# duxfrederic/lightcurver

Measured on AMD Instinct MI355X. Metric: cutouts/sec (PSF-fit + joint forward-model iter), 32x32 & 64x64 stamps, higher is better.
Workload: dtype f32

## Files before the change

lightcurver_amd/csrc/psf_kernels.h:

```cpp
#pragma once
#include <type_traits>
#include <utility>

#include "lc_common.h"
#include "starlet_device.h"

#ifndef LC_XPOLL_SLEEP
#define LC_XPOLL_SLEEP 2
#endif
#ifndef LC_P5_AHEAD
#define LC_P5_AHEAD 1
#endif
#ifndef LC_STARLET_LIVE_ADDR
#define LC_STARLET_LIVE_ADDR 1
#endif
#ifndef LC_SERIAL_TRIM
#define LC_SERIAL_TRIM 1
#endif
#ifndef LC_TASK_AHEAD
#define LC_TASK_AHEAD 1
#endif
#ifndef LC_V_ZERO_ONCE
#define LC_V_ZERO_ONCE LC_TASK_AHEAD
#endif
#ifndef LC_LOOP_ONLY
#define LC_LOOP_ONLY 1
#endif
#ifndef LC_LOOP_TOP_LIVE
#define LC_LOOP_TOP_LIVE 1
#endif
namespace lc {
constexpr int kXFlagStride = 16;

#ifdef LC_STAMPS
__device__ long long g_stamps[128];
#define LC_STAMP(k)                                                      \
  do {                                                                   \
    if ((blockIdx.x == 0 || blockIdx.x == 8) && threadIdx.x == 0 && it == A.n_iter - 1)  \
      g_stamps[(k) + (blockIdx.x == 8 ? 64 : 0)] = clock64();            \
  } while (0)
#else
#define LC_STAMP(k) do {} while (0)
#endif


struct PsfArgs {
  int F, S, n_iter, t0, hist_stride, mode;
  const float *data, *wgt;
  const float *W;
  const float *norms;
  const float *Tm;
  float *B, *mB, *sB;
  float *stars, *stars_m, *stars_s;
  float *hist;
  float *qscratch;
  float *out_loss, *out_chi2, *out_gstars, *out_ggrid, *out_gT, *out_model;
  float lam_sc, lam_hf;
  lc_adabelief_cfg ab;
  float *xch;
  int *xflags, *xabort;
  int launch_seq, heal, force_abort_it;
  const float *bkB, *bkmB, *bksB, *bkstars, *bkstars_m, *bkstars_s;
  int *heal_count;
  const float *ext_grad;
  const float *sched;
  float *B1, *mB1, *sB1;
  int xcd_fast;
};

typedef float lc_v4f __attribute__((ext_vector_type(4)));
__device__ __forceinline__ void store_sc1_x4(float *p, lc_v4f v) {
  asm volatile("global_store_dwordx4 %0, %1, off sc1\n\ts_nop 2" ::"v"(p), "v"(v) : "memory");
}
__device__ __forceinline__ void store_plain_x4(float *p, lc_v4f v) {
  asm volatile("global_store_dwordx4 %0, %1, off\n\ts_nop 2" ::"v"(p), "v"(v) : "memory");
}
__device__ __forceinline__ void store_sc1_f(float *p, float v) {
  asm volatile("global_store_dword %0, %1, off sc1" ::"v"(p), "v"(v) : "memory");
}
__device__ __forceinline__ void load_sc1_2x4(const float *p, lc_v4f &a, lc_v4f &b) {
  asm volatile("global_load_dwordx4 %0, %2, off sc1\n\tglobal_load_dwordx4 %1, %2, off offset:16 sc1\n\ts_waitcnt vmcnt(0)"
               : "=&v"(a), "=&v"(b)
               : "v"(p)
               : "memory");
}
__device__ __forceinline__ void load_sc1_2x4_1(const float *p, lc_v4f &a, lc_v4f &b, const float *ps, float &s) {
  asm volatile("global_load_dword %2, %4, off sc1\n\tglobal_load_dwordx4 %0, %3, off sc1\n\tglobal_load_dwordx4 %1, %3, off offset:16 sc1\n\ts_waitcnt vmcnt(0)"
               : "=&v"(a), "=&v"(b), "=&v"(s)
               : "v"(p), "v"(ps)
               : "memory");
}
__device__ __forceinline__ void load_sc1_x4(const float *p, lc_v4f &a) {
  asm volatile("global_load_dwordx4 %0, %1, off sc1\n\ts_waitcnt vmcnt(0)" : "=&v"(a) : "v"(p) : "memory");
}
__device__ __forceinline__ float load_sc1_f(const float *p) {
  float v;
  asm volatile("global_load_dword %0, %1, off sc1\n\ts_waitcnt vmcnt(0)" : "=&v"(v) : "v"(p) : "memory");
  return v;
}


template <int N_, int SS_, int PX_, int SG_, bool WC_ = false, int JB_ = 8>
struct PsfCfg {
  static constexpr int N = N_, SS = SS_, PX = PX_, SG = SG_;
  static constexpr bool WC = WC_;
  static constexpr bool SPLIT_LOOP_ONLY = (N == 32 || N == 64);
  static constexpr int n = N / SS;
  static constexpr int NTHR = N * N / PX;
  static constexpr int NW = (NTHR + kWave - 1) / kWave;
  static constexpr int NT = ntaps(SS);
  static constexpr int J = ilog2(N);
  static constexpr int LR = 8;
  static constexpr int LC = (JB_ * (N_ / SS_) / 4 >= 64) ? 4 : 2;
  static constexpr int LA = LC;
  static constexpr int TS = N + 1;
  static constexpr int RS = n + 1;
  static constexpr int OFF_T = 0;
  static constexpr int SZ_T = WC_ ? N * (N + 2 * (N / 4 + 10) + 1) : N * TS;
  static constexpr int OFF_R = OFF_T + SZ_T;
  static constexpr int SZ_R2 = SG * n * TS;
  static constexpr int VS = WC_ ? n + 3 : RS, VO = WC_ ? 1 : 0;
  static constexpr int SZ_V = SG * N * VS;
  static constexpr int JB = JB_;
  static constexpr int AP = N / 4 + 10;
  static constexpr int TSA = N + 2 * AP + 1;
  static constexpr int APR = AP / SS + 2;
  static constexpr int JBP = JB + 1;
  static constexpr int WSZ = JB * TSA + (n + 2 * APR) * JBP;
  static constexpr int SZ_VR = (SZ_V > StarletLds<N>::FLOATS) ? SZ_V : StarletLds<N>::FLOATS;
  static constexpr int OFF_WSC = OFF_R + SZ_VR;
  static constexpr int SZ_R = WC ? (SZ_VR + NW * WSZ) : ((2 * SZ_R2 > SZ_V) ? 2 * SZ_R2 : SZ_V);
  static constexpr int OFF_RES = OFF_R + SZ_R;
  static constexpr int SZ_RES = WC ? 0 : SG * n * n;
  static constexpr int OFF_TAPS = OFF_RES + SZ_RES;
  static constexpr int NTP = NT + 3;
  static constexpr int SZ_TAPS = (16 * 4 * NTP + 1) / 2 * 2 + 16 * 2 * NT * 2;
  static constexpr int OFF_TAPP = OFF_TAPS + (16 * 4 * NTP + 1) / 2 * 2;
  static constexpr int OFF_RED = OFF_TAPS + SZ_TAPS;
  static constexpr int IPS = n * n / LC;
  static constexpr int IPS_PAD = (IPS + kWave - 1) / kWave * kWave;
  static constexpr int SLOTS = IPS_PAD / kWave;
  static constexpr int SZ_REDX = 16 * NW;
  static constexpr int SZ_RED = (WC ? 16 * (n / JB) * 5 : SG * SLOTS * 5) + SZ_REDX + NW + 8;
  static constexpr int OFF_REDX = OFF_RED + (WC ? 16 * (n / JB) * 5 : SG * SLOTS * 5);
  static constexpr int OFF_REDW = OFF_REDX + SZ_REDX;
  static constexpr int OFF_STAR = OFF_RED + SZ_RED;
  static constexpr int MAXS = 16;
  static constexpr int SZ_STAR = MAXS * 20 + 16;
  static constexpr int LDS_FLOATS = OFF_STAR + SZ_STAR;
  static_assert(WC || StarletLds<N>::FLOATS <= SZ_T + SZ_R + SZ_RES, "starlet ping-pong buffers must fit over T + R + RES");
  static_assert(PX % SS == 0 && N % PX == 0 && n % LR == 0 && n % LC == 0 && n % LA == 0 && n % JB == 0, "tiling");
  static_assert(LDS_FLOATS * 4 <= 163840, "LDS");
  static_assert(OFF_TAPP % 2 == 0, "tap pairs are read as 64-bit words");
  static_assert(NTHR <= 1024 && NTHR % kWave == 0, "threads");
  static_assert(!WC_ || PX_ <= 8, "the WC layout keeps the pixel state in registers");
};


template <int SS, int NT>
__device__ inline void tap_entry(float delta, int k, float &tap, float &dtap, int &bq) {
  const int o = (int)nearbyintf(delta);
  const int base = o - kRg - (SS - 1);
  int q = base / SS;
  if (q * SS > base) --q;
  bq = q;
  const int m = q * SS + k;
  const float inv_s2 = 1.0f / (kSigmaG * kSigmaG);
  const float nrm = 0.3989422804014327f / kSigmaG;
  float a = 0.f, d = 0.f;
#pragma unroll
  for (int dv = 0; dv < SS; ++dv) {
    const int t = m + dv;
    if (t >= o - kRg && t <= o + kRg) {
      const float x = (float)t - delta;
      const float p = nrm * expf(-0.5f * x * x * inv_s2);
      a += p;
      d += p * x * inv_s2;
    }
  }
  tap = a;
  dtap = d;
}

template <class C, bool SPLIT = false>
__global__ __launch_bounds__(C::NTHR) void psf_fit_kernel(PsfArgs A) {
  constexpr int N = C::N, SS = C::SS, PX = C::PX, SG = C::SG, n = C::n, NT = C::NT, J = C::J;
  constexpr int NTHR = C::NTHR, TS = C::TS, RS = C::RS, LR = C::LR, LC = C::LC, LA = C::LA;
  extern __shared__ __align__(16) float lds[];
  float *T = lds + C::OFF_T;
  float *R2t = lds + C::OFF_R;
  float *R2xt = R2t + C::SZ_R2;
  float *V = lds + C::OFF_R;
  float *RES = lds + C::OFF_RES;
  float *TAPS = lds + C::OFF_TAPS + 1;
  constexpr int NTP = C::NTP;
  lc_v2f *TAPP = (lc_v2f *)(lds + C::OFF_TAPP);
  float *REDX = lds + C::OFF_REDX;
  float *RED = lds + C::OFF_RED;
  float *REDW = lds + C::OFF_REDW;
  float *SCAL = REDW + C::NW;
  float *SP = lds + C::OFF_STAR;
  float *SGR = SP + C::MAXS * 4;
  float *SM = SGR + C::MAXS * 5;
  float *SV = SM + C::MAXS * 4;
  int *BQ = (int *)(SV + C::MAXS * 4);

  int f = blockIdx.x, role = 0;
  if constexpr (SPLIT) {
    f = ((int)blockIdx.x >> 4) * 8 + ((int)blockIdx.x & 7);
    role = ((int)blockIdx.x >> 3) & 1;
    if (f >= A.F) return;
  }
  const bool conv_role = !SPLIT || role == 0, starlet_role = !SPLIT || role == 1;
  const int my_xcc = SPLIT ? (int)(__builtin_amdgcn_s_getreg(20 | (3 << 11)) & 15u) : 0;
  int same_xcd = 0;
  const int tid0 = threadIdx.x;
  const int S = A.S;
  constexpr bool LOOP_ONLY = SPLIT && LC_LOOP_ONLY && C::SPLIT_LOOP_ONLY;
  const bool loop = LOOP_ONLY || A.mode == 1;

  const float *dataf = A.data + (size_t)f * S * n * n;
  const float *wgtf = A.wgt + (size_t)f * S * n * n;

  if constexpr (!SPLIT) {
    if (A.heal) {
      if (__hip_atomic_load(A.xabort, __ATOMIC_RELAXED, __HIP_MEMORY_SCOPE_AGENT) != A.launch_seq) return;
      const size_t o = (size_t)f * N * N;
      for (int i = tid0; i < N * N; i += NTHR) {
        A.B[o + i] = A.bkB[o + i];
        A.mB[o + i] = A.bkmB[o + i];
        A.sB[o + i] = A.bksB[o + i];
      }
      if (tid0 < S * 4) {
        A.stars[(size_t)f * S * 4 + tid0] = A.bkstars[(size_t)f * S * 4 + tid0];
        A.stars_m[(size_t)f * S * 4 + tid0] = A.bkstars_m[(size_t)f * S * 4 + tid0];
        A.stars_s[(size_t)f * S * 4 + tid0] = A.bkstars_s[(size_t)f * S * 4 + tid0];
      }
      if (f == 0 && tid0 == 0) atomicAdd(A.heal_count, 1);
      __threadfence_block();
      __syncthreads();
    }
  }

  if constexpr (C::WC) {
    for (int i = tid0; i < C::SZ_T; i += NTHR) lds[C::OFF_T + i] = 0.f;
    for (int i = tid0; i < C::NW * C::WSZ; i += NTHR) lds[C::OFF_WSC + i] = 0.f;
  }
  if (tid0 < S * 4) {
    SP[tid0] = A.stars[(size_t)f * S * 4 + tid0];
    SM[tid0] = A.stars_m[(size_t)f * S * 4 + tid0];
    SV[tid0] = A.stars_s[(size_t)f * S * 4 + tid0];
  }
  __syncthreads();

  constexpr bool STATE_REGS = (PX <= 8);
  float *Bg = A.B, *mBg = A.mB, *sBg = A.sB;
  if constexpr (SPLIT && !STATE_REGS) {
    if (role == 1) {
      const size_t g0pix = (size_t)f * N * N + (size_t)(tid0 / (N / PX)) * N + (tid0 % (N / PX)) * PX;
#pragma unroll
      for (int q = 0; q < PX / 4; ++q) {
        ((float4 *)(A.B1 + g0pix))[q] = ((const float4 *)(A.B + g0pix))[q];
        ((float4 *)(A.mB1 + g0pix))[q] = ((const float4 *)(A.mB + g0pix))[q];
        ((float4 *)(A.sB1 + g0pix))[q] = ((const float4 *)(A.sB + g0pix))[q];
      }
      Bg = A.B1;
      mBg = A.mB1;
      sBg = A.sB1;
    }
  }
  float Bp[PX], Mp[PX], Sp_[PX], Tp[PX];
  {
    const size_t g0pix = (size_t)f * N * N + (size_t)(tid0 / (N / PX)) * N + (tid0 % (N / PX)) * PX;
#pragma unroll
    for (int q = 0; q < PX / 4; ++q) {
      if (STATE_REGS) {
        const float4 b = ((const float4 *)(A.B + g0pix))[q], t = ((const float4 *)(A.Tm + g0pix))[q];
        const float4 m = ((const float4 *)(A.mB + g0pix))[q], sv = ((const float4 *)(A.sB + g0pix))[q];
        Bp[4 * q] = b.x; Bp[4 * q + 1] = b.y; Bp[4 * q + 2] = b.z; Bp[4 * q + 3] = b.w;
        Tp[4 * q] = t.x; Tp[4 * q + 1] = t.y; Tp[4 * q + 2] = t.z; Tp[4 * q + 3] = t.w;
        Mp[4 * q] = m.x; Mp[4 * q + 1] = m.y; Mp[4 * q + 2] = m.z; Mp[4 * q + 3] = m.w;
        Sp_[4 * q] = sv.x; Sp_[4 * q + 1] = sv.y; Sp_[4 * q + 2] = sv.z; Sp_[4 * q + 3] = sv.w;
      }
    }
  }

  auto compute_taps = [&](int tid) {
    for (int e = tid; e < S * 2 * NTP; e += NTHR) {
      const int s = e / (2 * NTP), ax = (e / NTP) & 1, k = e % NTP - 1;
      float tap = 0.f, dtap = 0.f;
      int bq = 0;
      const float c_off = (N % 2 == 0) ? 0.5f : 0.0f;
      const float delta = fminf(fmaxf(SS * SP[s * 4 + 1 + ax], -(float)(N / 4)), (float)(N / 4)) + c_off;
      if (k >= 0 && k < NT) tap_entry<SS, NT>(delta, k, tap, dtap, bq);
      TAPS[(s * 4 + 2 * ax) * NTP + k] = tap;
      TAPS[(s * 4 + 2 * ax + 1) * NTP + k] = dtap;
      if (k >= 0 && k < NT) TAPP[(s * 2 + ax) * NT + k] = (lc_v2f){tap, dtap};
      if (k == 0) BQ[s * 2 + ax] = bq;
    }
  };
  auto step_stars = [&](int tid) {
#pragma clang fp contract(off)
    if (tid < S * 3) {
      const float lr = SCAL[0], bc1 = SCAL[1], bc2 = SCAL[2];
      const float b1 = A.ab.b1, b2 = A.ab.b2, eps = A.ab.eps, eps_root = A.ab.eps_root;
      const int s = tid / 3, q = tid % 3;
      const float g = SGR[s * 5 + 1 + q];
      const float mn = b1 * SM[s * 4 + q] + (1.f - b1) * g;
      const float dg = g - mn;
      const float sn = b2 * SV[s * 4 + q] + (1.f - b2) * dg * dg + eps_root;
      SM[s * 4 + q] = mn;
      SV[s * 4 + q] = sn;
      SP[s * 4 + q] -= lr * (mn * bc1) / (sqrtf(sn * bc2) + eps);
    }
  };
  auto update_stars_and_taps = [&](int tid) {
    step_stars(tid);
    __syncthreads();
    compute_taps(tid);
  };
  if (conv_role) compute_taps(tid0);
  constexpr bool TRIM = SPLIT && C::WC && PX == 8 && LC_SERIAL_TRIM;
  static_assert(!TRIM || 3 * C::MAXS <= kWave, "the x0 sums and the stars' step are lanes of one wave");
  [[maybe_unused]] float tpix_next[TRIM ? PX : 1];
  constexpr bool C2_SPLIT = SPLIT && C::WC && PX == 8;
  constexpr bool TASK_AHEAD = C2_SPLIT && LC_TASK_AHEAD, V_ZERO_ONCE = C2_SPLIT && LC_V_ZERO_ONCE;
  constexpr bool TOP_LIVE = C2_SPLIT && LOOP_ONLY && LC_LOOP_TOP_LIVE;
  if constexpr (V_ZERO_ONCE) {
    if (role == 0) {
      for (int i = tid0; i < SG * N; i += NTHR) {
        V[i * C::VS] = 0.f;
        V[i * C::VS + n + 1] = 0.f;
      }
    }
  }
  if constexpr (TRIM) {
    if (role == 0) {
      const int pu = tid0 / (N / PX), pv = (tid0 % (N / PX)) * PX;
#pragma unroll
      for (int p = 0; p < PX; ++p) {
        tpix_next[p] = Bp[p] + Tp[p];
        T[pu * C::TSA + C::AP + pv + p] = tpix_next[p];
      }
    }
    __syncthreads();
  }
  for (int it = 0; it < A.n_iter; ++it) {
    const int tglob = A.t0 + it;
    if constexpr (SPLIT) {
      if (A.force_abort_it == it && f == 0 && role == 1) {
        if (tid0 == 0) __hip_atomic_store(A.xabort, A.launch_seq, __ATOMIC_RELAXED, __HIP_MEMORY_SCOPE_AGENT);
        break;
      }
    }
    int tid = tid0;
    LC_LAUNDER(tid);
    const int lane = tid & 63, wid = tid >> 6;
    const int pu = tid / (N / PX);
    const int pv = (tid % (N / PX)) * PX;
    const size_t gpix = (size_t)f * N * N + (size_t)pu * N + pv;
    const int tid_c = TOP_LIVE ? tid0 : tid, lane_c = tid_c & 63, wid_c = tid_c >> 6;
    const int pu_c = tid_c / (N / PX), pv_c = (tid_c % (N / PX)) * PX;
    if (tid < 3 && loop) SCAL[tid] = A.sched[3 * tglob + tid];
    LC_STAMP(0);
    float gB[PX];
#pragma unroll
    for (int p = 0; p < PX; ++p) gB[p] = 0.f;
    float tpix[PX];
    if (conv_role) {
    if constexpr (TRIM) {
#pragma unroll
      for (int p = 0; p < PX; ++p) tpix[p] = tpix_next[p];
    } else if (C::WC && STATE_REGS) {
#pragma unroll
      for (int p = 0; p < PX; ++p) {
        tpix[p] = Bp[p] + Tp[p];
        T[pu_c * C::TSA + C::AP + pv_c + p] = tpix[p];
      }
    } else if (STATE_REGS) {
#pragma unroll
      for (int p = 0; p < PX; ++p) T[pu_c * TS + pv_c + p] = Bp[p] + Tp[p];
    } else {
      const float4 *bp = (const float4 *)(Bg + gpix);
      const float4 *tp = (const float4 *)(A.Tm + gpix);
#pragma unroll
      for (int q = 0; q < PX / 4; ++q) {
        const float4 b = bp[q], t = tp[q];
        T[pu_c * TS + pv_c + 4 * q + 0] = b.x + t.x;
        T[pu_c * TS + pv_c + 4 * q + 1] = b.y + t.y;
        T[pu_c * TS + pv_c + 4 * q + 2] = b.z + t.z;
        T[pu_c * TS + pv_c + 4 * q + 3] = b.w + t.w;
      }
    }
    if constexpr (!TOP_LIVE)
      if (tid_c < S * 5) SGR[tid_c] = 0.f;

    for (int g0 = 0; g0 < S; g0 += SG) {
      if (!TRIM || g0 > 0) __syncthreads();
      LC_STAMP(1 + 5 * (g0 / SG));
      if constexpr (C::WC) {
        constexpr int JB = C::JB, NBLK = n / JB;
        float *wsc = lds + C::OFF_WSC + wid_c * C::WSZ;
        constexpr int TSA = C::TSA, AP = C::AP, APR = C::APR;
        float *R2w = wsc + AP, *RESw = wsc + JB * TSA + APR * C::JBP;
        if constexpr (TASK_AHEAD) {
          static_assert(SS == 2 && N == kWave && JB * (n / LC) == kWave && LA == LC, "one item per lane in each pass of a task");
          constexpr int NP = (NT + 1) / 2, WL2 = (JB - 1) + NP, WL = SS * (LC - 1) + NT, WI = (SS * LA - 1 + NT - 1) / SS + 1;
          const int jl = lane_c % JB, a0 = (lane_c / JB) * LC;
          const int ntask = min(SG, S - g0) * NBLK;
          float dpre[LC], wpre[LC];
          lc_v2f tr2[NP], win2[WL2];
          lc_v2f py[NP];
          float rv[WI];
          auto pixel_request = [&](int task) {
            const int s = g0 + task / NBLK, jd0 = (task % NBLK) * JB;
#pragma unroll
            for (int j = 0; j < LC; ++j) {
              const size_t pix = (size_t)s * n * n + (size_t)(a0 + j) * n + jd0 + jl;
              dpre[j] = dataf[pix];
              wpre[j] = wgtf[pix];
            }
          };
          auto row_request = [&](int task, int bqx) {
            const int s = g0 + task / NBLK, jd0 = (task % NBLK) * JB;
            const float *tx = TAPS + (s * 4 + 0) * NTP;
#pragma unroll
            for (int h = 0; h < NP; ++h) tr2[h] = (lc_v2f){tx[NT - 1 - 2 * h], tx[NT - 2 - 2 * h]};
            const float *trow = T + lane_c * TSA + AP + SS * (jd0 - bqx) - (NT - 1);
#pragma unroll
            for (int i = 0; i < WL2; ++i) win2[i] = (lc_v2f){trow[2 * i], trow[2 * i + 1]};
          };
          auto row_fma_store = [&] {
            lc_v2f acc[JB];
#pragma unroll
            for (int j = 0; j < JB; ++j) acc[j] = (lc_v2f){0.f, 0.f};
#pragma unroll
            for (int h = 0; h < NP; ++h) {
#pragma unroll
              for (int j = 0; j < JB; ++j) acc[j] = pk_fma(tr2[h], win2[j + h], acc[j]);
            }
#pragma unroll
            for (int j = 0; j < JB; ++j) R2w[j * TSA + lane_c] = acc[j].x + acc[j].y;
          };
          auto tcol_request = [&](int task, int bqy) {
            const float *ty = TAPS + ((g0 + task / NBLK) * 4 + 2) * NTP;
#pragma unroll
            for (int q = 0; q < NP; ++q) py[q] = (lc_v2f){ty[2 * q], ty[2 * q - 1]};
            const float *rcol = RESw + (bqy + a0) * C::JBP + jl;
#pragma unroll
            for (int i = 0; i < WI; ++i) rv[i] = rcol[i * C::JBP];
          };
          auto tcol_fma_store = [&](int task) {
            const int sl = task / NBLK, jd0 = (task % NBLK) * JB;
            lc_v2f out2[LA];
#pragma unroll
            for (int h = 0; h < LA; ++h) out2[h] = (lc_v2f){0.f, 0.f};
#pragma unroll
            for (int i = 0; i < WI; ++i) {
              const lc_v2f rr = pk_bcast(rv[i]);
#pragma unroll
              for (int h = 0; h < LA; ++h)
                if (i - h >= 0 && i - h < NP) out2[h] = pk_fma(py[i - h], rr, out2[h]);
            }
            float *vrow = V + (sl * N + SS * a0) * C::VS + C::VO + jd0 + jl;
#pragma unroll
            for (int h = 0; h < LA; ++h) {
              vrow[(2 * h) * C::VS] = out2[h].x;
              vrow[(2 * h + 1) * C::VS] = out2[h].y;
            }
            if constexpr (!V_ZERO_ONCE) {
              if (jd0 + jl == 0) {
#pragma unroll
                for (int r = 0; r < SS * LA; ++r) V[(sl * N + SS * a0 + r) * C::VS] = 0.f;
              }
              if (jd0 + jl == n - 1) {
#pragma unroll
                for (int r = 0; r < SS * LA; ++r) V[(sl * N + SS * a0 + r) * C::VS + n + 1] = 0.f;
              }
            }
          };
// ... 492 lines not shown
              const lc_v2f vv = pk_bcast(use.vwin[i]);
#pragma unroll
              for (int k = 0; k < NT; ++k) {
                const int rel = SS * i - k;
                if (rel >= 0 && rel < PX) accp[rel] = pk_fma(use.txd[k], vv, accp[rel]);
              }
            }
            float gxs = 0.f;
#pragma unroll
            for (int p = 0; p < PX; ++p) {
              gB[p] = fmaf(use.amp, accp[p].x, gB[p]);
              gxs = fmaf(accp[p].y, tpix[p], gxs);
            }
            gxs = wave_sum(gxs);
            if (lane_c == 0) REDX[s * C::NW + wid_c] = gxs;
          };
          auto nothing = [] {};
          auto p5_window = [&](int sl, P5Ops &o, int bq) {
            o.amp = SP[(g0 + sl) * 4 + 0];
            const float *vrow = V + (sl * N + pu_c) * C::VS + 1;
            const int jd0 = bq + pv_c / SS;
#pragma unroll
            for (int i = 0; i < WJ; ++i) o.vwin[i] = vrow[min(max(jd0 + i, -1), n)];
            __builtin_amdgcn_sched_barrier(0);
          };
          auto p5_taps = [&](int sl, P5Ops &o) {
            __builtin_amdgcn_sched_barrier(0);
#pragma unroll
            for (int k = 0; k < NT; ++k) o.txd[k] = TAPP[((g0 + sl) * 2 + 0) * NT + k];
            __builtin_amdgcn_sched_barrier(0);
          };
          const int ns = min(SG, S - g0);
          P5Ops opsA, opsB;
          int bqn = BQ[min(g0 + 1, S - 1) * 2 + 0];
          p5_window(0, opsA, BQ[g0 * 2 + 0]);
          p5_taps(0, opsA);
          int sl = 0;
#pragma clang loop unroll(disable)
          while (sl + 1 < ns) {
            progress_prio((4 * sl) / SG);
            const int bqnn = BQ[min(g0 + sl + 2, S - 1) * 2 + 0];
            p5_window(sl + 1, opsB, bqn);
            p5_star(sl, opsA, [&] { p5_taps(sl + 1, opsB); });
            if (sl + 2 >= ns) {
              opsA = opsB;
              sl += 1;
              break;
            }
            bqn = BQ[min(g0 + sl + 3, S - 1) * 2 + 0];
            p5_window(sl + 2, opsA, bqnn);
            p5_star(sl + 1, opsB, [&] { p5_taps(sl + 2, opsA); });
            sl += 2;
          }
          progress_prio((4 * sl) / SG);
          p5_star(sl, opsA, nothing);
        } else {
          for (int sl = 0; sl < SG; ++sl) {
            const int s = g0 + sl;
            if (s >= S) break;
            progress_prio((4 * sl) / SG);
            const int bq = BQ[s * 2 + 0];
            const float amp = SP[s * 4 + 0];
            lc_v2f txd[NT];
#pragma unroll
            for (int k = 0; k < NT; ++k) txd[k] = TAPP[(s * 2 + 0) * NT + k];
            lc_v2f accp[PX];
#pragma unroll
            for (int p = 0; p < PX; ++p) accp[p] = (lc_v2f){0.f, 0.f};
            const float *vrow = V + (sl * N + pu_c) * C::VS + 1;
            const int jd0 = bq + pv_c / SS;
            float vwin[WJ];
#pragma unroll
            for (int i = 0; i < WJ; ++i) vwin[i] = vrow[min(max(jd0 + i, -1), n)];
#pragma unroll
            for (int i = 0; i < WJ; ++i) {
              const lc_v2f vv = pk_bcast(vwin[i]);
#pragma unroll
              for (int k = 0; k < NT; ++k) {
                const int rel = SS * i - k;
                if (rel >= 0 && rel < PX) accp[rel] = pk_fma(txd[k], vv, accp[rel]);
              }
            }
            float gxs = 0.f;
#pragma unroll
            for (int p = 0; p < PX; ++p) {
              gB[p] = fmaf(amp, accp[p].x, gB[p]);
              gxs = fmaf(accp[p].y, tpix[p], gxs);
            }
            gxs = wave_sum(gxs);
            if (lane_c == 0) REDX[s * C::NW + wid_c] = gxs;
          }
        }
        __builtin_amdgcn_s_setprio(0);
      } else {
        constexpr int WJ = (PX - 1 + NT - 1) / SS + 1;
        for (int sl = 0; sl < SG; ++sl) {
          const int s = g0 + sl;
          if (s >= S) break;
          const float *tx = TAPS + (s * 4 + 0) * NTP, *dtx = tx + NTP;
          const int bq = BQ[s * 2 + 0];
          const float amp = SP[s * 4 + 0];
          float acc[PX], gxs = 0.f;
#pragma unroll
          for (int p = 0; p < PX; ++p) acc[p] = 0.f;
#pragma unroll
          for (int i = 0; i < WJ; ++i) {
            const int jd = i + bq + pv_c / SS;
            const int ci = min(max(jd, 0), n - 1);
            float vv = V[(sl * N + pu_c) * RS + ci];
            vv = (jd >= 0 && jd < n) ? vv : 0.f;
            float dsum = 0.f;
#pragma unroll
            for (int k = 0; k < NT; ++k) {
              const int rel = SS * i - k;
              if (rel >= 0 && rel < PX) {
                acc[rel] = fmaf(tx[k], vv, acc[rel]);
                dsum = fmaf(dtx[k], T[pu_c * TS + pv_c + rel], dsum);
              }
            }
            gxs = fmaf(vv, dsum, gxs);
          }
#pragma unroll
          for (int p = 0; p < PX; ++p) gB[p] = fmaf(amp, acc[p], gB[p]);
          gxs = wave_sum(gxs);
          if (lane_c == 0) REDX[s * C::NW + wid_c] = gxs;
        }
      }
      LC_STAMP(17);
    }
    if (A.ext_grad) {
#pragma unroll
      for (int p = 0; p < PX; ++p) gB[p] += A.ext_grad[gpix + p];
    }
    }
    if constexpr (TRIM) {
      if (role == 0) {
        LC_STAMP(41);
        float *mine = A.xch + (((size_t)f * 2 + (it & 1)) * 2 + 0) * (N * N + 64);
#pragma unroll
        for (int q = 0; q < PX / 4; ++q) {
          lc_v4f v;
          v.x = gB[4 * q];
          v.y = gB[4 * q + 1];
          v.z = gB[4 * q + 2];
          v.w = gB[4 * q + 3];
          if (same_xcd) store_plain_x4(mine + pu_c * N + pv_c + 4 * q, v);
          else store_sc1_x4(mine + pu_c * N + pv_c + 4 * q, v);
        }
        if (tid_c == 0 && it == 0) store_sc1_f(mine + N * N + 1, __int_as_float(my_xcc + 1));
      }
    }
    __syncthreads();
    LC_STAMP(40);
    {
      if (conv_role && tid < S) {
        float acc = 0.f;
#pragma unroll
        for (int w = 0; w < C::NW; ++w) acc += REDX[tid * C::NW + w];
        SGR[tid * 5 + 2] = acc * SP[tid * 4 + 0] * SS;
      }
    }

    if constexpr (!LOOP_ONLY) {
      if (A.out_gT) {
#pragma unroll
        for (int p = 0; p < PX; ++p) A.out_gT[gpix + p] = gB[p];
      }
    }

    float l1 = 0.f;
    float z[PX];
#pragma unroll
    for (int p = 0; p < PX; ++p) z[p] = 0.f;
    if (starlet_role && (LOOP_ONLY || A.lam_sc != 0.f || A.lam_hf != 0.f)) {
      float bpix[PX];
      if (STATE_REGS) {
#pragma unroll
        for (int p = 0; p < PX; ++p) bpix[p] = Bp[p];
      } else {
        const float4 *bp = (const float4 *)(Bg + gpix);
#pragma unroll
        for (int q = 0; q < PX / 4; ++q) {
          const float4 b = bp[q];
          bpix[4 * q] = b.x;
          bpix[4 * q + 1] = b.y;
          bpix[4 * q + 2] = b.z;
          bpix[4 * q + 3] = b.w;
        }
      }
      constexpr bool LIVE_ADDR = SPLIT && STATE_REGS && LC_STARLET_LIVE_ADDR;
      starlet_l1_grad<N, PX, ilog2(N), LIVE_ADDR>(bpix, A.W ? A.W + (size_t)f * J * N * N : nullptr, A.norms,
                                                  A.qscratch + (size_t)f * J * N * N, A.lam_sc, A.lam_hf,
                                                  C::WC ? lds + C::OFF_R : lds, tid, l1, z);
    }
    LC_STAMP(42);
    if (!TRIM || role == 1) {
      {
        const float wl = wave_sum(l1);
        if (lane == 0) REDW[wid] = wl;
      }
      __syncthreads();
    }
    float tl1 = 0.f;
    if (tid == 0 && starlet_role)
      for (int w = 0; w < C::NW; ++w) tl1 += REDW[w];
    LC_STAMP(44);
    if constexpr (SPLIT) {
      constexpr int XS = N * N + 64;
      float *mine = A.xch + (((size_t)f * 2 + (it & 1)) * 2 + role) * XS;
      const float *theirs = A.xch + (((size_t)f * 2 + (it & 1)) * 2 + (1 - role)) * XS;
      const int poff = pu * N + pv;
      if (!TRIM || role == 1) {
#pragma unroll
      for (int q = 0; q < PX / 4; ++q) {
        lc_v4f v;
        v.x = role ? z[4 * q] : gB[4 * q];
        v.y = role ? z[4 * q + 1] : gB[4 * q + 1];
        v.z = role ? z[4 * q + 2] : gB[4 * q + 2];
        v.w = role ? z[4 * q + 3] : gB[4 * q + 3];
        if (same_xcd) store_plain_x4(mine + poff + 4 * q, v);
        else store_sc1_x4(mine + poff + 4 * q, v);
      }
      if (tid == 0 && role == 1) {
        if (same_xcd) asm volatile("global_store_dword %0, %1, off" ::"v"(mine + N * N), "v"(tl1) : "memory");
        else store_sc1_f(mine + N * N, tl1);
      }
      if (tid == 0 && it == 0) store_sc1_f(mine + N * N + 1, __int_as_float(my_xcc + 1));
      }
      constexpr bool TAPS_LATE = STATE_REGS;
      if (role == 0 && loop) {
        if constexpr (TRIM) wave_lds_sync();
        if (TAPS_LATE) step_stars(tid);
        else update_stars_and_taps(tid);
      }
      asm volatile("s_waitcnt vmcnt(0)" ::: "memory");
      __syncthreads();
      LC_STAMP(45);
      int *OK = (int *)(SCAL + 5);
      if (tid == 0) {
        if (same_xcd) asm volatile("global_store_dword %0, %1, off" ::"v"(A.xflags + ((size_t)f * 2 + role) * kXFlagStride), "v"(it + 1) : "memory");
        else __hip_atomic_store(A.xflags + ((size_t)f * 2 + role) * kXFlagStride, it + 1, __ATOMIC_RELAXED, __HIP_MEMORY_SCOPE_AGENT);
        int ok = 1, spins = 0;
        while (__hip_atomic_load(A.xflags + ((size_t)f * 2 + (1 - role)) * kXFlagStride, __ATOMIC_RELAXED, __HIP_MEMORY_SCOPE_AGENT) < it + 1) {
          __builtin_amdgcn_s_sleep(LC_XPOLL_SLEEP);
          ++spins;
          if (spins > (1 << 21) ||
              ((spins & 255) == 0 && __hip_atomic_load(A.xabort, __ATOMIC_RELAXED, __HIP_MEMORY_SCOPE_AGENT) == A.launch_seq)) {
            __hip_atomic_store(A.xabort, A.launch_seq, __ATOMIC_RELAXED, __HIP_MEMORY_SCOPE_AGENT);
            ok = 0;
            break;
          }
        }
        if (it == 0 && ok) OK[1] = (A.xcd_fast && __float_as_int(load_sc1_f(theirs + N * N + 1)) == my_xcc + 1) ? 1 : 0;
        *OK = ok;
#ifdef LC_XCH_ACQUIRE
        __builtin_amdgcn_fence(__ATOMIC_ACQUIRE, "agent");
        asm volatile("s_waitcnt vmcnt(0)" ::: "memory");
#endif
      }
      if (TAPS_LATE && role == 0 && loop) compute_taps((tid + NTHR / 2) % NTHR);
      __syncthreads();
      LC_STAMP(46);
      if (*OK == 0) break;
      if (it == 0) same_xcd = OK[1];
      float other[PX];
      float tl1_other = 0.f;
      if constexpr (PX == 8) {
        lc_v4f a, b;
        load_sc1_2x4_1(theirs + poff, a, b, theirs + N * N, tl1_other);
        other[0] = a.x; other[1] = a.y; other[2] = a.z; other[3] = a.w;
        other[4] = b.x; other[5] = b.y; other[6] = b.z; other[7] = b.w;
      } else {
#pragma unroll
        for (int q = 0; q < PX / 4; ++q) {
          lc_v4f a;
          load_sc1_x4(theirs + poff + 4 * q, a);
          other[4 * q] = a.x; other[4 * q + 1] = a.y; other[4 * q + 2] = a.z; other[4 * q + 3] = a.w;
        }
      }
#pragma unroll
      for (int p = 0; p < PX; ++p) {
        if (role) gB[p] = other[p]; else z[p] = other[p];
      }
      if (tid == 0 && role == 0) tl1 = (PX == 8) ? tl1_other : load_sc1_f(theirs + N * N);
      LC_STAMP(47);
    }
    if (!TRIM && tid == 0 && conv_role) {
      float chi = 0.f;
      for (int s = 0; s < S; ++s) chi += SGR[s * 5];
      const float loss = 0.5f * chi + tl1;
      A.hist[(size_t)f * A.hist_stride + tglob] = loss;
      if constexpr (!LOOP_ONLY) {
        if (A.out_loss) A.out_loss[f] = loss;
        if (A.out_chi2) A.out_chi2[f] = chi;
      }
    }
    if constexpr (!LOOP_ONLY) {
      if (A.out_ggrid) {
#pragma unroll
        for (int p = 0; p < PX; ++p) A.out_ggrid[gpix + p] = gB[p] + z[p];
      }
      if (A.out_gstars && tid < S * 4) {
        const int s = tid / 4, q = tid % 4;
        A.out_gstars[(size_t)f * S * 4 + tid] = SGR[s * 5 + 1 + q];
      }
    }
    if (loop) {
#pragma clang fp contract(off)
      const float lr = SCAL[0], bc1 = SCAL[1], bc2 = SCAL[2];
      const float b1 = A.ab.b1, b2 = A.ab.b2, eps = A.ab.eps, eps_root = A.ab.eps_root;
      if (STATE_REGS) {
#pragma unroll
        for (int p = 0; p < PX; ++p) {
          const float g = gB[p] + z[p];
          const float mn = b1 * Mp[p] + (1.f - b1) * g;
          const float dg = g - mn;
          const float sn = b2 * Sp_[p] + (1.f - b2) * dg * dg + eps_root;
          Mp[p] = mn;
          Sp_[p] = sn;
          Bp[p] -= lr * (mn * bc1) * __builtin_amdgcn_rcpf(__builtin_amdgcn_sqrtf(sn * bc2) + eps);
        }
      }
      if constexpr (!STATE_REGS) {
        float4 *bp = (float4 *)(Bg + gpix);
        float4 *mp = (float4 *)(mBg + gpix);
        float4 *sp = (float4 *)(sBg + gpix);
        float4 bq[PX / 4], mq[PX / 4], sq[PX / 4];
#pragma unroll
        for (int q = 0; q < PX / 4; ++q) {
          bq[q] = bp[q];
          mq[q] = mp[q];
          sq[q] = sp[q];
        }
#pragma unroll
        for (int q = 0; q < PX / 4; ++q) {
          float *bb = &bq[q].x, *mm = &mq[q].x, *ss_ = &sq[q].x;
#pragma unroll
          for (int e = 0; e < 4; ++e) {
            const float g = gB[4 * q + e] + z[4 * q + e];
            const float mn = b1 * mm[e] + (1.f - b1) * g;
            const float dg = g - mn;
            const float sn = b2 * ss_[e] + (1.f - b2) * dg * dg + eps_root;
            mm[e] = mn;
            ss_[e] = sn;
            bb[e] -= lr * (mn * bc1) * __builtin_amdgcn_rcpf(__builtin_amdgcn_sqrtf(sn * bc2) + eps);
          }
        }
#pragma unroll
        for (int q = 0; q < PX / 4; ++q) {
          bp[q] = bq[q];
          mp[q] = mq[q];
          sp[q] = sq[q];
        }
      }
      if constexpr (!SPLIT) update_stars_and_taps(tid);
    }
    if constexpr (TRIM) {
      if (role == 0) {
#pragma unroll
        for (int p = 0; p < PX; ++p) {
          tpix_next[p] = Bp[p] + Tp[p];
          T[pu_c * C::TSA + C::AP + pv_c + p] = tpix_next[p];
        }
        if (tid_c == 0) {
          float chi = 0.f;
          for (int s = 0; s < S; ++s) chi += SGR[s * 5];
          const float loss = 0.5f * chi + tl1;
          A.hist[(size_t)f * A.hist_stride + tglob] = loss;
          if constexpr (!LOOP_ONLY) {
            if (A.out_loss) A.out_loss[f] = loss;
            if (A.out_chi2) A.out_chi2[f] = chi;
          }
        }
      }
    }
    __syncthreads();
    LC_STAMP(43);
  }

  if (loop && STATE_REGS && conv_role) {
    const size_t g0pix = (size_t)f * N * N + (size_t)(tid0 / (N / PX)) * N + (tid0 % (N / PX)) * PX;
#pragma unroll
    for (int q = 0; q < PX / 4; ++q) {
      ((float4 *)(A.B + g0pix))[q] = make_float4(Bp[4 * q], Bp[4 * q + 1], Bp[4 * q + 2], Bp[4 * q + 3]);
      ((float4 *)(A.mB + g0pix))[q] = make_float4(Mp[4 * q], Mp[4 * q + 1], Mp[4 * q + 2], Mp[4 * q + 3]);
      ((float4 *)(A.sB + g0pix))[q] = make_float4(Sp_[4 * q], Sp_[4 * q + 1], Sp_[4 * q + 2], Sp_[4 * q + 3]);
    }
  }
  if (loop && tid0 < S * 4 && conv_role) {
    A.stars[(size_t)f * S * 4 + tid0] = SP[tid0];
    A.stars_m[(size_t)f * S * 4 + tid0] = SM[tid0];
    A.stars_s[(size_t)f * S * 4 + tid0] = SV[tid0];
// ... 5 lines not shown
```

lightcurver_amd/csrc/starlet_device.h:

```cpp
#pragma once
#include <utility>

#include "lc_common.h"

namespace lc {

__device__ __forceinline__ void progress_prio(int k) {
#ifndef LC_NO_PROGRESS_PRIO
  if (k <= 0) __builtin_amdgcn_s_setprio(3);
  else if (k == 1) __builtin_amdgcn_s_setprio(2);
  else if (k == 2) __builtin_amdgcn_s_setprio(1);
  else __builtin_amdgcn_s_setprio(0);
#endif
}
__device__ __forceinline__ void progress_prio_end(int done, int total) {
#ifndef LC_NO_PROGRESS_PRIO
  const int left = total - 1 - done;
  if (left >= 3) __builtin_amdgcn_s_setprio(3);
  else if (left == 2) __builtin_amdgcn_s_setprio(2);
  else if (left == 1) __builtin_amdgcn_s_setprio(1);
  else __builtin_amdgcn_s_setprio(0);
#endif
}

// ... 410 lines not shown
template <int LPR>
__device__ __forceinline__ float swz_line_last(float v) {
  constexpr int pat = ((~(LPR - 1)) & 0x1F) | ((LPR - 1) << 5);
  return __builtin_bit_cast(float, __builtin_amdgcn_ds_swizzle(__builtin_bit_cast(int, v), pat));
}
#define LC_TAP1(a, o, c, dir, k) \
  "v_fmac_f32_dpp %" #a ", %" #o ", %" #c " " dir ":%" #k " row_mask:0xf bank_mask:0xf bound_ctrl:1\n\t"
#define LC_TAP2(c, dir, k) LC_TAP1(0, 2, c, dir, k) LC_TAP1(1, 3, c, dir, k)
#define LC_TAP4(c, dir, k) LC_TAP1(0, 4, c, dir, k) LC_TAP1(1, 5, c, dir, k) LC_TAP1(2, 6, c, dir, k) LC_TAP1(3, 7, c, dir, k)
#define LC_TAP8(c, dir, k)                                                                                        \
  LC_TAP1(0, 8, c, dir, k) LC_TAP1(1, 9, c, dir, k) LC_TAP1(2, 10, c, dir, k) LC_TAP1(3, 11, c, dir, k)             \
  LC_TAP1(4, 12, c, dir, k) LC_TAP1(5, 13, c, dir, k) LC_TAP1(6, 14, c, dir, k) LC_TAP1(7, 15, c, dir, k)
#define LC_MUL1(w, o, c, dir) "v_mul_f32_dpp %" #w ", %" #o ", %" #c " " dir ":1 row_mask:0xf bank_mask:0xf bound_ctrl:1\n\t"
template <int K1, int K2>
__device__ __forceinline__ void dpp_taps(float (&acc)[2], const float (&own)[2], float cl1, float cu1, float cl2, float cu2) {
  asm("s_nop 1\n\t" LC_TAP2(4, "row_shr", 8) LC_TAP2(5, "row_shl", 8) LC_TAP2(6, "row_shr", 9) LC_TAP2(7, "row_shl", 9)
      : "+v"(acc[0]), "+v"(acc[1])
      : "v"(own[0]), "v"(own[1]), "v"(cl1), "v"(cu1), "v"(cl2), "v"(cu2), "n"(K1), "n"(K2));
}
template <int K1>
__device__ __forceinline__ void dpp_taps(float (&acc)[2], const float (&own)[2], float cl1, float cu1) {
  asm("s_nop 1\n\t" LC_TAP2(4, "row_shr", 6) LC_TAP2(5, "row_shl", 6)
      : "+v"(acc[0]), "+v"(acc[1])
      : "v"(own[0]), "v"(own[1]), "v"(cl1), "v"(cu1), "n"(K1));
}
template <int K1, int K2>
__device__ __forceinline__ void dpp_taps(float (&acc)[4], const float (&own)[4], float cl1, float cu1, float cl2, float cu2) {
  asm("s_nop 1\n\t" LC_TAP4(8, "row_shr", 12) LC_TAP4(9, "row_shl", 12) LC_TAP4(10, "row_shr", 13) LC_TAP4(11, "row_shl", 13)
      : "+v"(acc[0]), "+v"(acc[1]), "+v"(acc[2]), "+v"(acc[3])
      : "v"(own[0]), "v"(own[1]), "v"(own[2]), "v"(own[3]), "v"(cl1), "v"(cu1), "v"(cl2), "v"(cu2), "n"(K1), "n"(K2));
}
template <int K1>
__device__ __forceinline__ void dpp_taps(float (&acc)[4], const float (&own)[4], float cl1, float cu1) {
  asm("s_nop 1\n\t" LC_TAP4(8, "row_shr", 10) LC_TAP4(9, "row_shl", 10)
      : "+v"(acc[0]), "+v"(acc[1]), "+v"(acc[2]), "+v"(acc[3])
      : "v"(own[0]), "v"(own[1]), "v"(own[2]), "v"(own[3]), "v"(cl1), "v"(cu1), "n"(K1));
}
template <int K1, int K2>
__device__ __forceinline__ void dpp_taps(float (&acc)[8], const float (&own)[8], float cl1, float cu1, float cl2, float cu2) {
  asm("s_nop 1\n\t" LC_TAP8(16, "row_shr", 20) LC_TAP8(17, "row_shl", 20) LC_TAP8(18, "row_shr", 21) LC_TAP8(19, "row_shl", 21)
      : "+v"(acc[0]), "+v"(acc[1]), "+v"(acc[2]), "+v"(acc[3]), "+v"(acc[4]), "+v"(acc[5]), "+v"(acc[6]), "+v"(acc[7])
      : "v"(own[0]), "v"(own[1]), "v"(own[2]), "v"(own[3]), "v"(own[4]), "v"(own[5]), "v"(own[6]), "v"(own[7]), "v"(cl1),
        "v"(cu1), "v"(cl2), "v"(cu2), "n"(K1), "n"(K2));
}
template <int K1>
__device__ __forceinline__ void dpp_taps(float (&acc)[8], const float (&own)[8], float cl1, float cu1) {
  asm("s_nop 1\n\t" LC_TAP8(16, "row_shr", 18) LC_TAP8(17, "row_shl", 18)
      : "+v"(acc[0]), "+v"(acc[1]), "+v"(acc[2]), "+v"(acc[3]), "+v"(acc[4]), "+v"(acc[5]), "+v"(acc[6]), "+v"(acc[7])
      : "v"(own[0]), "v"(own[1]), "v"(own[2]), "v"(own[3]), "v"(own[4]), "v"(own[5]), "v"(own[6]), "v"(own[7]), "v"(cl1),
        "v"(cu1), "n"(K1));
}
template <bool SHR>
__device__ __forceinline__ void dpp_gated(float *w, const float *in, float gate, std::integral_constant<int, 2>) {
  if constexpr (SHR)
    asm("s_nop 1\n\t" LC_MUL1(0, 2, 4, "row_shr") LC_MUL1(1, 3, 4, "row_shr") : "=&v"(w[0]), "=&v"(w[1]) : "v"(in[0]), "v"(in[1]), "v"(gate));
  else
    asm("s_nop 1\n\t" LC_MUL1(0, 2, 4, "row_shl") LC_MUL1(1, 3, 4, "row_shl") : "=&v"(w[0]), "=&v"(w[1]) : "v"(in[0]), "v"(in[1]), "v"(gate));
}
#define LC_MUL4(dir) LC_MUL1(0, 4, 8, dir) LC_MUL1(1, 5, 8, dir) LC_MUL1(2, 6, 8, dir) LC_MUL1(3, 7, 8, dir)
template <bool SHR>
__device__ __forceinline__ void dpp_gated(float *w, const float *in, float gate, std::integral_constant<int, 4>) {
  if constexpr (SHR)
    asm("s_nop 1\n\t" LC_MUL4("row_shr") : "=&v"(w[0]), "=&v"(w[1]), "=&v"(w[2]), "=&v"(w[3]) : "v"(in[0]), "v"(in[1]), "v"(in[2]), "v"(in[3]), "v"(gate));
  else
    asm("s_nop 1\n\t" LC_MUL4("row_shl") : "=&v"(w[0]), "=&v"(w[1]), "=&v"(w[2]), "=&v"(w[3]) : "v"(in[0]), "v"(in[1]), "v"(in[2]), "v"(in[3]), "v"(gate));
}
#undef LC_MUL4
#define LC_MUL8(dir)                                                                                \
  LC_MUL1(0, 8, 16, dir) LC_MUL1(1, 9, 16, dir) LC_MUL1(2, 10, 16, dir) LC_MUL1(3, 11, 16, dir)       \
  LC_MUL1(4, 12, 16, dir) LC_MUL1(5, 13, 16, dir) LC_MUL1(6, 14, 16, dir) LC_MUL1(7, 15, 16, dir)
#define LC_MUL8_OPS                                                                                                      \
  : "=&v"(w[0]), "=&v"(w[1]), "=&v"(w[2]), "=&v"(w[3]), "=&v"(w[4]), "=&v"(w[5]), "=&v"(w[6]), "=&v"(w[7])                 \
  : "v"(in[0]), "v"(in[1]), "v"(in[2]), "v"(in[3]), "v"(in[4]), "v"(in[5]), "v"(in[6]), "v"(in[7]), "v"(gate)
template <bool SHR>
__device__ __forceinline__ void dpp_gated(float *w, const float *in, float gate, std::integral_constant<int, 8>) {
  if constexpr (SHR) asm("s_nop 1\n\t" LC_MUL8("row_shr") LC_MUL8_OPS);
  else asm("s_nop 1\n\t" LC_MUL8("row_shl") LC_MUL8_OPS);
}
#undef LC_MUL8_OPS
#undef LC_MUL8
#undef LC_MUL1
#undef LC_TAP8
#undef LC_TAP4
#undef LC_TAP2
#undef LC_TAP1

template <int N, int PX, int LPR, int D, bool ADJ>
__device__ __forceinline__ void line_pass(const float (&own)[PX], const LineLane &L, float (&out)[PX]) {
  constexpr float b0 = 0.375f, b1 = 0.25f, b2 = 0.0625f;
  const int lil = L.lil;
  if constexpr (D >= PX) {
    constexpr int K1 = D / PX, K2 = 2 * D / PX;
    const float cl1 = (K1 < LPR && lil >= K1) ? b1 : 0.f, cu1 = (K1 < LPR && lil + K1 < LPR) ? b1 : 0.f;
    const float cl2 = (K2 < LPR && lil >= K2) ? b2 : 0.f, cu2 = (K2 < LPR && lil + K2 < LPR) ? b2 : 0.f;
    const float ef = ((lil < K1) ? b1 : 0.f) + ((lil < K2) ? b2 : 0.f);
    const float el = ((lil + K1 >= LPR) ? b1 : 0.f) + ((lil + K2 >= LPR) ? b2 : 0.f);
    float e = 0.f;
    if constexpr (!ADJ) e = fmaf(ef, swz_line_first<LPR>(own[0]), el * swz_line_last<LPR>(own[PX - 1]));
#pragma unroll
    for (int p = 0; p < PX; ++p) out[p] = fmaf(b0, own[p], e);
    if constexpr (K2 < LPR) dpp_taps<K1, K2>(out, own, cl1, cu1, cl2, cu2);
    else if constexpr (K1 < LPR) dpp_taps<K1>(out, own, cl1, cu1);
    if constexpr (ADJ) {
      float full = own[0];
#pragma unroll
      for (int p = 1; p < PX; ++p) full += own[p];
      const float hs = line_sum<LPR>(full * ef), ts = line_sum<LPR>(full * el);
      out[0] = fmaf(L.is_first, hs, out[0]);
      out[PX - 1] = fmaf(L.is_last, ts, out[PX - 1]);
    }
  } else {
    static_assert(2 * D <= PX, "dilations below PX reach the adjacent lane only");
    const float has_lower = 1.f - L.is_first, has_upper = 1.f - L.is_last;
    float w[3 * PX];
#pragma unroll
    for (int q = 0; q < PX; ++q) {
      w[q] = 0.f;
      w[PX + q] = own[q];
      w[2 * PX + q] = 0.f;
    }
    dpp_gated<true>(&w[PX - 2 * D], &own[PX - 2 * D], has_lower, std::integral_constant<int, 2 * D>{});
    dpp_gated<false>(&w[2 * PX], &own[0], has_upper, std::integral_constant<int, 2 * D>{});
#pragma unroll
    for (int p = 0; p < PX; ++p) {
      float acc = b0 * own[p];
      acc = fmaf(b1, w[PX + p - D] + w[PX + p + D], acc);
      acc = fmaf(b2, w[PX + p - 2 * D] + w[PX + p + 2 * D], acc);
      out[p] = acc;
    }
    if constexpr (!ADJ) {
      const float cf = L.is_first * own[0], cl = L.is_last * own[PX - 1];
#pragma unroll
      for (int p = 0; p < 2 * D; ++p) {
        out[p] = fmaf((p < D) ? b1 + b2 : b2, cf, out[p]);
        out[PX - 1 - p] = fmaf((p < D) ? b1 + b2 : b2, cl, out[PX - 1 - p]);
      }
    } else {
      float h1 = 0.f, h2 = 0.f, t1 = 0.f, t2 = 0.f;
#pragma unroll
      for (int p = 0; p < 2 * D; ++p) {
        if (p < D) {
          h1 += own[p];
          t1 += own[PX - 1 - p];
        }
        h2 += own[p];
        t2 += own[PX - 1 - p];
      }
      out[0] = fmaf(L.is_first, fmaf(b1, h1, b2 * h2), out[0]);
      out[PX - 1] = fmaf(L.is_last, fmaf(b1, t1, b2 * t2), out[PX - 1]);
    }
  }
}

template <int N, int PX, int JUSE, bool LIVE_ADDR = false>
__device__ __forceinline__ void starlet_l1_grad_dpp(const float img[PX], const float *Wf, const float *norms, float *qscr,
                                                    float lam_sc, float lam_hf, float *lds, int tid, float &l1,
                                                    float z[PX]) {
  constexpr int J = JUSE, TS = StarletLds<N>::TS, LPR = N / PX;
  float *bufA = lds, *bufB = lds + N * TS;
  const int pu_ = tid / LPR, pv_ = (tid % LPR) * PX;
  const int cv_ = tid / LPR, cu0_ = (tid % LPR) * PX;
  const int rb_ = pu_ * TS + pv_, cb_ = cu0_ * TS + cv_;
  const size_t wo_ = (size_t)pu_ * N + pv_;
  LineLane L;
  L.lil = tid % LPR;
  L.is_first = (L.lil == 0) ? 1.f : 0.f;
  L.is_last = (L.lil == LPR - 1) ? 1.f : 0.f;
  l1 = 0.f;
  constexpr bool QREG = (J * PX <= 64);
  float qreg[QREG ? J : 1][PX];
  float c[PX];
#pragma unroll
  for (int p = 0; p < PX; ++p) {
    c[p] = img[p];
    z[p] = 0.f;
  }
  auto transpose_offsets = [&](int &rb, int &cb) {
    if constexpr (LIVE_ADDR) {
      rb = rb_;
      cb = cb_;
    } else {
      int pu = pu_, pv = pv_, cu0 = cu0_, cv = cv_;
      LC_LAUNDER(pu);
      LC_LAUNDER(pv);
      LC_LAUNDER(cu0);
      LC_LAUNDER(cv);
      rb = pu * TS + pv;
      cb = cu0 * TS + cv;
    }
  };
  auto to_columns = [&](const float (&v)[PX], float (&o)[PX]) {
    int rb, cb;
    transpose_offsets(rb, cb);
#pragma unroll
    for (int p = 0; p < PX; ++p) bufA[rb + p] = v[p];
    __syncthreads();
#pragma unroll
    for (int p = 0; p < PX; ++p) o[p] = bufA[cb + p * TS];
  };
  auto to_rows = [&](const float (&v)[PX], float (&o)[PX]) {
    int rb, cb;
    transpose_offsets(rb, cb);
#pragma unroll
    for (int p = 0; p < PX; ++p) bufB[cb + p * TS] = v[p];
    __syncthreads();
#pragma unroll
    for (int p = 0; p < PX; ++p) o[p] = bufB[rb + p];
  };
  static_for(std::make_integer_sequence<int, J>{}, [&](auto jc) {
    constexpr int j = decltype(jc)::value, d = 1 << j;
    float wj[PX];
    if (Wf) {
      size_t wo = wo_;
      if constexpr (!LIVE_ADDR) {
        int pu = pu_, pv = pv_;
        LC_LAUNDER(pu);
        LC_LAUNDER(pv);
        wo = (size_t)pu * N + pv;
      }
      const float4 *wp = (const float4 *)(Wf + (size_t)j * N * N + wo);
#pragma unroll
      for (int q = 0; q < PX / 4; ++q) {
        const float4 w4 = wp[q];
        wj[4 * q] = w4.x;
        wj[4 * q + 1] = w4.y;
        wj[4 * q + 2] = w4.z;
        wj[4 * q + 3] = w4.w;
      }
    } else {
      const float nv = norms[j];
#pragma unroll
      for (int p = 0; p < PX; ++p) wj[p] = nv;
    }
    float r[PX], rc[PX], cc[PX], cn[PX];
    line_pass<N, PX, LPR, d, false>(c, L, r);
    to_columns(r, rc);
    line_pass<N, PX, LPR, d, false>(rc, L, cc);
    to_rows(cc, cn);
    const float lam = (j == 0) ? lam_hf : lam_sc;
    float q[PX];
#pragma unroll
    for (int p = 0; p < PX; ++p) {
      const float w = c[p] - cn[p];
      const float lw = lam * wj[p];
      l1 = fmaf(lw, fabsf(w), l1);
      q[p] = (w > 0.f) ? lw : ((w < 0.f) ? -lw : 0.f);
      c[p] = cn[p];
    }
    if constexpr (QREG) {
#pragma unroll
      for (int p = 0; p < PX; ++p) qreg[j][p] = q[p];
    } else {
      float4 *qp = (float4 *)(qscr + (size_t)j * N * N + (size_t)pu_ * N + pv_);
#pragma unroll
      for (int qq = 0; qq < PX / 4; ++qq) qp[qq] = make_float4(q[4 * qq], q[4 * qq + 1], q[4 * qq + 2], q[4 * qq + 3]);
    }
  });
  static_for(std::make_integer_sequence<int, J>{}, [&](auto jc) {
    constexpr int j = J - 1 - decltype(jc)::value, d = 1 << j;
    float q[PX];
    if constexpr (QREG) {
#pragma unroll
      for (int p = 0; p < PX; ++p) q[p] = qreg[j][p];
    } else {
      const float4 *qp = (const float4 *)(qscr + (size_t)j * N * N + (size_t)pu_ * N + pv_);
#pragma unroll
      for (int qq = 0; qq < PX / 4; ++qq) {
        const float4 v4 = qp[qq];
        q[4 * qq] = v4.x;
        q[4 * qq + 1] = v4.y;
        q[4 * qq + 2] = v4.z;
        q[4 * qq + 3] = v4.w;
      }
    }
    float y[PX], rt[PX], yc[PX], ct[PX], back[PX];
#pragma unroll
    for (int p = 0; p < PX; ++p) y[p] = z[p] - q[p];
    line_pass<N, PX, LPR, d, true>(y, L, rt);
    to_columns(rt, yc);
    line_pass<N, PX, LPR, d, true>(yc, L, ct);
    to_rows(ct, back);
#pragma unroll
    for (int p = 0; p < PX; ++p) z[p] = q[p] + back[p];
  });
}

template <int N, int PX, int JUSE = ilog2(N), bool LIVE_ADDR = false>
__device__ __forceinline__ void starlet_l1_grad(const float img[PX], const float *Wf, const float *norms, float *qscr,
                                                float lam_sc, float lam_hf, float *lds, int tid, float &l1,
                                                float z[PX]) {
  constexpr int LPR = N / PX;
  if constexpr ((LPR == 4 || LPR == 8 || LPR == 16) && PX >= 2 && PX <= 8)
    starlet_l1_grad_dpp<N, PX, JUSE, LIVE_ADDR>(img, Wf, norms, qscr, lam_sc, lam_hf, lds, tid, l1, z);
  else
    starlet_l1_grad_lds<N, PX, JUSE>(img, Wf, norms, qscr, lam_sc, lam_hf, lds, tid, l1, z);
}

}
```

Baseline: 65.97 million.

## Store role-1 starlet gradient before the L1 reduction barrier and fuse stars step

```diff
diff --git a/lightcurver_amd/csrc/psf_kernels.h b/lightcurver_amd/csrc/psf_kernels.h
--- a/lightcurver_amd/csrc/psf_kernels.h
+++ b/lightcurver_amd/csrc/psf_kernels.h
@@ -29,6 +29,12 @@
 #ifndef LC_LOOP_TOP_LIVE
 #define LC_LOOP_TOP_LIVE 1
 #endif
+#ifndef LC_R1_STORE_FIRST
+#define LC_R1_STORE_FIRST 1
+#endif
+#ifndef LC_STARS_ONE_TRIP
+#define LC_STARS_ONE_TRIP 1
+#endif
 namespace lc {
 constexpr int kXFlagStride = 16;
 
@@ -74,6 +80,14 @@
 }
 __device__ __forceinline__ void store_plain_x4(float *p, lc_v4f v) {
   asm volatile("global_store_dwordx4 %0, %1, off\n\ts_nop 2" ::"v"(p), "v"(v) : "memory");
+}
+template <int OFF>
+__device__ __forceinline__ void store_sc1_x4_at(float *base, unsigned byte_off, lc_v4f v) {
+  asm volatile("global_store_dwordx4 %0, %1, %2 offset:%3 sc1\n\ts_nop 2" ::"v"(byte_off), "v"(v), "s"(base), "n"(OFF) : "memory");
+}
+template <int OFF>
+__device__ __forceinline__ void store_plain_x4_at(float *base, unsigned byte_off, lc_v4f v) {
+  asm volatile("global_store_dwordx4 %0, %1, %2 offset:%3\n\ts_nop 2" ::"v"(byte_off), "v"(v), "s"(base), "n"(OFF) : "memory");
 }
 __device__ __forceinline__ void store_sc1_f(float *p, float v) {
   asm volatile("global_store_dword %0, %1, off sc1" ::"v"(p), "v"(v) : "memory");
@@ -326,6 +340,37 @@
   constexpr bool C2_SPLIT = SPLIT && C::WC && PX == 8;
   constexpr bool TASK_AHEAD = C2_SPLIT && LC_TASK_AHEAD, V_ZERO_ONCE = C2_SPLIT && LC_V_ZERO_ONCE;
   constexpr bool TOP_LIVE = C2_SPLIT && LOOP_ONLY && LC_LOOP_TOP_LIVE;
+  constexpr bool R1_STORE_FIRST = C2_SPLIT && LC_R1_STORE_FIRST;
+  constexpr bool STARS_ONE_TRIP = TRIM && LC_STARS_ONE_TRIP;
+  auto x0_sums_and_step_stars = [&](int tid, bool step) {
+#pragma clang fp contract(off)
+    if (tid < S * 3) {
+      const int s = tid / 3, q = tid % 3;
+      float part[C::NW];
+#pragma unroll
+      for (int w = 0; w < C::NW; ++w) part[w] = REDX[s * C::NW + w];
+      const float amp = SP[s * 4 + 0];
+      const float gq = SGR[s * 5 + 1 + (q == 1 ? 0 : q)];
+      const float lr = SCAL[0], bc1 = SCAL[1], bc2 = SCAL[2];
+      const float m0 = SM[s * 4 + q], s0 = SV[s * 4 + q], p0 = SP[s * 4 + q];
+      __builtin_amdgcn_sched_barrier(0);
+      float acc = 0.f;
+#pragma unroll
+      for (int w = 0; w < C::NW; ++w) acc += part[w];
+      const float gx = acc * amp * SS;
+      if (q == 1) SGR[s * 5 + 2] = gx;
+      if (step) {
+        const float b1 = A.ab.b1, b2 = A.ab.b2, eps = A.ab.eps, eps_root = A.ab.eps_root;
+        const float g = (q == 1) ? gx : gq;
+        const float mn = b1 * m0 + (1.f - b1) * g;
+        const float dg = g - mn;
+        const float sn = b2 * s0 + (1.f - b2) * dg * dg + eps_root;
+        SM[s * 4 + q] = mn;
+        SV[s * 4 + q] = sn;
+        SP[s * 4 + q] = p0 - lr * (mn * bc1) / (sqrtf(sn * bc2) + eps);
+      }
+    }
+  };
   if constexpr (V_ZERO_ONCE) {
     if (role == 0) {
       for (int i = tid0; i < SG * N; i += NTHR) {
@@ -1124,7 +1169,7 @@
     }
     __syncthreads();
     LC_STAMP(40);
-    {
+    if constexpr (!STARS_ONE_TRIP) {
       if (conv_role && tid < S) {
         float acc = 0.f;
 #pragma unroll
@@ -1161,12 +1206,31 @@
         }
       }
       constexpr bool LIVE_ADDR = SPLIT && STATE_REGS && LC_STARLET_LIVE_ADDR;
-      starlet_l1_grad<N, PX, ilog2(N), LIVE_ADDR>(bpix, A.W ? A.W + (size_t)f * J * N * N : nullptr, A.norms,
+      starlet_l1_grad<N, PX, ilog2(N), LIVE_ADDR, R1_STORE_FIRST>(bpix, A.W ? A.W + (size_t)f * J * N * N : nullptr, A.norms,
                                                   A.qscratch + (size_t)f * J * N * N, A.lam_sc, A.lam_hf,
                                                   C::WC ? lds + C::OFF_R : lds, tid, l1, z);
     }
     LC_STAMP(42);
-    if (!TRIM || role == 1) {
+    const bool r1_first = R1_STORE_FIRST && role == 1;
+    if constexpr (R1_STORE_FIRST) {
+      if (role == 1) {
+        float *mine = A.xch + (((size_t)f * 2 + (it & 1)) * 2 + 1) * (N * N + 64);
+        static_assert(!R1_STORE_FIRST || PX == 8, "two quads per thread");
+        const unsigned boff = (unsigned)(pu * N + pv) * 4u;
+        const lc_v4f v0 = {z[0], z[1], z[2], z[3]}, v1 = {z[4], z[5], z[6], z[7]};
+        if (same_xcd) {
+          store_plain_x4_at<0>(mine, boff, v0);
+          store_plain_x4_at<16>(mine, boff, v1);
+        } else {
+          store_sc1_x4_at<0>(mine, boff, v0);
+          store_sc1_x4_at<16>(mine, boff, v1);
+        }
+        if (tid == 0 && it == 0) store_sc1_f(mine + N * N + 1, __int_as_float(my_xcc + 1));
+        const float wl = wave_sum(l1);
+        if (lane == 0) REDW[wid] = wl;
+      }
+    }
+    if ((!TRIM || role == 1) && !r1_first) {
       {
         const float wl = wave_sum(l1);
         if (lane == 0) REDW[wid] = wl;
@@ -1174,7 +1238,7 @@
       __syncthreads();
     }
     float tl1 = 0.f;
-    if (tid == 0 && starlet_role)
+    if (tid == 0 && starlet_role && !r1_first)
       for (int w = 0; w < C::NW; ++w) tl1 += REDW[w];
     LC_STAMP(44);
     if constexpr (SPLIT) {
@@ -1182,7 +1246,7 @@
       float *mine = A.xch + (((size_t)f * 2 + (it & 1)) * 2 + role) * XS;
       const float *theirs = A.xch + (((size_t)f * 2 + (it & 1)) * 2 + (1 - role)) * XS;
       const int poff = pu * N + pv;
-      if (!TRIM || role == 1) {
+      if ((!TRIM || role == 1) && !r1_first) {
 #pragma unroll
       for (int q = 0; q < PX / 4; ++q) {
         lc_v4f v;
@@ -1200,7 +1264,9 @@
       if (tid == 0 && it == 0) store_sc1_f(mine + N * N + 1, __int_as_float(my_xcc + 1));
       }
       constexpr bool TAPS_LATE = STATE_REGS;
-      if (role == 0 && loop) {
+      if constexpr (STARS_ONE_TRIP) {
+        if (role == 0) x0_sums_and_step_stars(tid, loop);
+      } else if (role == 0 && loop) {
         if constexpr (TRIM) wave_lds_sync();
         if (TAPS_LATE) step_stars(tid);
         else update_stars_and_taps(tid);
@@ -1210,6 +1276,12 @@
       LC_STAMP(45);
       int *OK = (int *)(SCAL + 5);
       if (tid == 0) {
+        if (r1_first) {
+          for (int w = 0; w < C::NW; ++w) tl1 += REDW[w];
+          if (same_xcd) asm volatile("global_store_dword %0, %1, off" ::"v"(mine + N * N), "v"(tl1) : "memory");
+          else store_sc1_f(mine + N * N, tl1);
+          asm volatile("s_waitcnt vmcnt(0)" ::: "memory");
+        }
         if (same_xcd) asm volatile("global_store_dword %0, %1, off" ::"v"(A.xflags + ((size_t)f * 2 + role) * kXFlagStride), "v"(it + 1) : "memory");
         else __hip_atomic_store(A.xflags + ((size_t)f * 2 + role) * kXFlagStride, it + 1, __ATOMIC_RELAXED, __HIP_MEMORY_SCOPE_AGENT);
         int ok = 1, spins = 0;
diff --git a/lightcurver_amd/csrc/starlet_device.h b/lightcurver_amd/csrc/starlet_device.h
--- a/lightcurver_amd/csrc/starlet_device.h
+++ b/lightcurver_amd/csrc/starlet_device.h
@@ -586,7 +586,7 @@
   }
 }
 
-template <int N, int PX, int JUSE, bool LIVE_ADDR = false>
+template <int N, int PX, int JUSE, bool LIVE_ADDR = false, bool L1_IN_PLACE = false>
 __device__ __forceinline__ void starlet_l1_grad_dpp(const float img[PX], const float *Wf, const float *norms, float *qscr,
                                                     float lam_sc, float lam_hf, float *lds, int tid, float &l1,
                                                     float z[PX]) {
@@ -681,6 +681,7 @@
       q[p] = (w > 0.f) ? lw : ((w < 0.f) ? -lw : 0.f);
       c[p] = cn[p];
     }
+    if constexpr (L1_IN_PLACE) asm volatile("" : "+v"(l1));
     if constexpr (QREG) {
 #pragma unroll
       for (int p = 0; p < PX; ++p) qreg[j][p] = q[p];
@@ -719,13 +720,13 @@
   });
 }
 
-template <int N, int PX, int JUSE = ilog2(N), bool LIVE_ADDR = false>
+template <int N, int PX, int JUSE = ilog2(N), bool LIVE_ADDR = false, bool L1_IN_PLACE = false>
 __device__ __forceinline__ void starlet_l1_grad(const float img[PX], const float *Wf, const float *norms, float *qscr,
                                                 float lam_sc, float lam_hf, float *lds, int tid, float &l1,
                                                 float z[PX]) {
   constexpr int LPR = N / PX;
   if constexpr ((LPR == 4 || LPR == 8 || LPR == 16) && PX >= 2 && PX <= 8)
-    starlet_l1_grad_dpp<N, PX, JUSE, LIVE_ADDR>(img, Wf, norms, qscr, lam_sc, lam_hf, lds, tid, l1, z);
+    starlet_l1_grad_dpp<N, PX, JUSE, LIVE_ADDR, L1_IN_PLACE>(img, Wf, norms, qscr, lam_sc, lam_hf, lds, tid, l1, z);
   else
     starlet_l1_grad_lds<N, PX, JUSE>(img, Wf, norms, qscr, lam_sc, lam_hf, lds, tid, l1, z);
 }
```

Result: no change. 66.35 million, median of 6 (+0.6%).
